# XuyangBai/D3Feat

Measured on NVIDIA H100. Metric: points/sec through KPFCNN encoder, higher is better.
Workload: dtype f32

## Files before the change

d3feat_b200/csrc/tc_common.cuh:

```cuda
#pragma once
#include "common.cuh"

namespace d3f {

__device__ __forceinline__ uint32_t smem_u32(const void* p) { return (uint32_t)__cvta_generic_to_shared(p); }

__device__ __forceinline__ void mbar_init(uint32_t bar, uint32_t count) {
  asm volatile("mbarrier.init.shared::cta.b64 [%0], %1;" ::"r"(bar), "r"(count) : "memory");
}
__device__ __forceinline__ void mbar_arrive(uint32_t bar) {
  asm volatile("mbarrier.arrive.shared::cta.b64 _, [%0];" ::"r"(bar) : "memory");
}
__device__ __forceinline__ void mbar_wait(uint32_t bar, uint32_t parity) {
  uint32_t ok;
  do {
    asm volatile(
        "{\n\t.reg .pred p;\n\t"
        "mbarrier.try_wait.parity.shared::cta.b64 p, [%1], %2;\n\t"
        "selp.u32 %0, 1, 0, p;\n\t}"
        : "=r"(ok)
        : "r"(bar), "r"(parity)
        : "memory");
  } while (!ok);
}
__device__ __forceinline__ void fence_proxy_async() { asm volatile("fence.proxy.async.shared::cta;" ::: "memory"); }

__device__ __forceinline__ uint64_t make_smem_desc(uint32_t saddr) {
  uint64_t d = 0;
  d |= (uint64_t)((saddr >> 4) & 0x3FFF);
  d |= (uint64_t)1 << 16;
  d |= (uint64_t)(1024 >> 4) << 32;
  d |= (uint64_t)1 << 62;
  return d;
}

__device__ __forceinline__ void wgmma_fence() { asm volatile("wgmma.fence.sync.aligned;" ::: "memory"); }
__device__ __forceinline__ void wgmma_commit() { asm volatile("wgmma.commit_group.sync.aligned;" ::: "memory"); }
template <int N>
__device__ __forceinline__ void wgmma_wait() { asm volatile("wgmma.wait_group.sync.aligned %0;" ::"n"(N) : "memory"); }
template <int R>
__device__ __forceinline__ void wgmma_reg_fence(float* d) {
#pragma unroll
  for (int i = 0; i < R; ++i) asm volatile("" : "+f"(d[i])::"memory");
}

template <int N>
__device__ __forceinline__ void wgmma_tf32(float* d, uint64_t adesc, uint64_t bdesc);
template <>
__device__ __forceinline__ void wgmma_tf32<32>(float* d, uint64_t adesc, uint64_t bdesc) {
  asm volatile(
      "{\n\t.reg .pred p;\n\tsetp.ne.b32 p, %18, 0;\n\t"
      "wgmma.mma_async.sync.aligned.m64n32k8.f32.tf32.tf32 "
      "{%0, %1, %2, %3, %4, %5, %6, %7, %8, %9, %10, %11, %12, %13, %14, %15}, %16, %17, p, 1, 1;\n\t}"
      : "+f"(d[0]), "+f"(d[1]), "+f"(d[2]), "+f"(d[3]), "+f"(d[4]), "+f"(d[5]), "+f"(d[6]), "+f"(d[7]), "+f"(d[8]), "+f"(d[9]), "+f"(d[10]), "+f"(d[11]), "+f"(d[12]), "+f"(d[13]), "+f"(d[14]), "+f"(d[15])
      : "l"(adesc), "l"(bdesc), "r"(1)
      : "memory");
}
template <>
__device__ __forceinline__ void wgmma_tf32<64>(float* d, uint64_t adesc, uint64_t bdesc) {
  asm volatile(
      "{\n\t.reg .pred p;\n\tsetp.ne.b32 p, %34, 0;\n\t"
      "wgmma.mma_async.sync.aligned.m64n64k8.f32.tf32.tf32 "
      "{%0, %1, %2, %3, %4, %5, %6, %7, %8, %9, %10, %11, %12, %13, %14, %15, %16, %17, %18, %19, %20, %21, %22, %23, %24, %25, %26, %27, %28, %29, %30, %31}, %32, %33, p, 1, 1;\n\t}"
      : "+f"(d[0]), "+f"(d[1]), "+f"(d[2]), "+f"(d[3]), "+f"(d[4]), "+f"(d[5]), "+f"(d[6]), "+f"(d[7]), "+f"(d[8]), "+f"(d[9]), "+f"(d[10]), "+f"(d[11]), "+f"(d[12]), "+f"(d[13]), "+f"(d[14]), "+f"(d[15]), "+f"(d[16]), "+f"(d[17]), "+f"(d[18]), "+f"(d[19]), "+f"(d[20]), "+f"(d[21]), "+f"(d[22]), "+f"(d[23]), "+f"(d[24]), "+f"(d[25]), "+f"(d[26]), "+f"(d[27]), "+f"(d[28]), "+f"(d[29]), "+f"(d[30]), "+f"(d[31])
      : "l"(adesc), "l"(bdesc), "r"(1)
      : "memory");
}
template <>
__device__ __forceinline__ void wgmma_tf32<96>(float* d, uint64_t adesc, uint64_t bdesc) {
  asm volatile(
      "{\n\t.reg .pred p;\n\tsetp.ne.b32 p, %50, 0;\n\t"
      "wgmma.mma_async.sync.aligned.m64n96k8.f32.tf32.tf32 "
      "{%0, %1, %2, %3, %4, %5, %6, %7, %8, %9, %10, %11, %12, %13, %14, %15, %16, %17, %18, %19, %20, %21, %22, %23, %24, %25, %26, %27, %28, %29, %30, %31, %32, %33, %34, %35, %36, %37, %38, %39, %40, %41, %42, %43, %44, %45, %46, %47}, %48, %49, p, 1, 1;\n\t}"
      : "+f"(d[0]), "+f"(d[1]), "+f"(d[2]), "+f"(d[3]), "+f"(d[4]), "+f"(d[5]), "+f"(d[6]), "+f"(d[7]), "+f"(d[8]), "+f"(d[9]), "+f"(d[10]), "+f"(d[11]), "+f"(d[12]), "+f"(d[13]), "+f"(d[14]), "+f"(d[15]), "+f"(d[16]), "+f"(d[17]), "+f"(d[18]), "+f"(d[19]), "+f"(d[20]), "+f"(d[21]), "+f"(d[22]), "+f"(d[23]), "+f"(d[24]), "+f"(d[25]), "+f"(d[26]), "+f"(d[27]), "+f"(d[28]), "+f"(d[29]), "+f"(d[30]), "+f"(d[31]), "+f"(d[32]), "+f"(d[33]), "+f"(d[34]), "+f"(d[35]), "+f"(d[36]), "+f"(d[37]), "+f"(d[38]), "+f"(d[39]), "+f"(d[40]), "+f"(d[41]), "+f"(d[42]), "+f"(d[43]), "+f"(d[44]), "+f"(d[45]), "+f"(d[46]), "+f"(d[47])
      : "l"(adesc), "l"(bdesc), "r"(1)
      : "memory");
}
template <>
__device__ __forceinline__ void wgmma_tf32<128>(float* d, uint64_t adesc, uint64_t bdesc) {
  asm volatile(
      "{\n\t.reg .pred p;\n\tsetp.ne.b32 p, %66, 0;\n\t"
      "wgmma.mma_async.sync.aligned.m64n128k8.f32.tf32.tf32 "
      "{%0, %1, %2, %3, %4, %5, %6, %7, %8, %9, %10, %11, %12, %13, %14, %15, %16, %17, %18, %19, %20, %21, %22, %23, %24, %25, %26, %27, %28, %29, %30, %31, %32, %33, %34, %35, %36, %37, %38, %39, %40, %41, %42, %43, %44, %45, %46, %47, %48, %49, %50, %51, %52, %53, %54, %55, %56, %57, %58, %59, %60, %61, %62, %63}, %64, %65, p, 1, 1;\n\t}"
      : "+f"(d[0]), "+f"(d[1]), "+f"(d[2]), "+f"(d[3]), "+f"(d[4]), "+f"(d[5]), "+f"(d[6]), "+f"(d[7]), "+f"(d[8]), "+f"(d[9]), "+f"(d[10]), "+f"(d[11]), "+f"(d[12]), "+f"(d[13]), "+f"(d[14]), "+f"(d[15]), "+f"(d[16]), "+f"(d[17]), "+f"(d[18]), "+f"(d[19]), "+f"(d[20]), "+f"(d[21]), "+f"(d[22]), "+f"(d[23]), "+f"(d[24]), "+f"(d[25]), "+f"(d[26]), "+f"(d[27]), "+f"(d[28]), "+f"(d[29]), "+f"(d[30]), "+f"(d[31]), "+f"(d[32]), "+f"(d[33]), "+f"(d[34]), "+f"(d[35]), "+f"(d[36]), "+f"(d[37]), "+f"(d[38]), "+f"(d[39]), "+f"(d[40]), "+f"(d[41]), "+f"(d[42]), "+f"(d[43]), "+f"(d[44]), "+f"(d[45]), "+f"(d[46]), "+f"(d[47]), "+f"(d[48]), "+f"(d[49]), "+f"(d[50]), "+f"(d[51]), "+f"(d[52]), "+f"(d[53]), "+f"(d[54]), "+f"(d[55]), "+f"(d[56]), "+f"(d[57]), "+f"(d[58]), "+f"(d[59]), "+f"(d[60]), "+f"(d[61]), "+f"(d[62]), "+f"(d[63])
      : "l"(adesc), "l"(bdesc), "r"(1)
      : "memory");
}

__device__ __forceinline__ float4 lds128(uint32_t addr) {
  float4 v;
  asm volatile("ld.shared.v4.f32 {%0, %1, %2, %3}, [%4];" : "=f"(v.x), "=f"(v.y), "=f"(v.z), "=f"(v.w) : "r"(addr));
  return v;
}
__device__ __forceinline__ void sts128(uint32_t addr, float4 v) {
  asm volatile("st.shared.v4.f32 [%0], {%1, %2, %3, %4};" ::"r"(addr), "f"(v.x), "f"(v.y), "f"(v.z), "f"(v.w) : "memory");
}
__device__ __forceinline__ float lds32(uint32_t addr) {
  float v;
  asm volatile("ld.shared.f32 %0, [%1];" : "=f"(v) : "r"(addr));
  return v;
}
__device__ __forceinline__ void sts32(uint32_t addr, float v) {
  asm volatile("st.shared.f32 [%0], %1;" ::"r"(addr), "f"(v) : "memory");
}

__device__ __forceinline__ void split_tf32(float x, float& hi, float& lo) {
  hi = __uint_as_float((__float_as_uint(x) + 0x1000u) & 0xFFFFE000u);
  lo = x - hi;
}

__device__ __forceinline__ void tma_bulk_g2s(uint32_t dst_smem, const void* src, uint32_t bytes, uint32_t bar) {
  asm volatile("cp.async.bulk.shared::cluster.global.mbarrier::complete_tx::bytes [%0], [%1], %2, [%3];"
               ::"r"(dst_smem), "l"(src), "r"(bytes), "r"(bar) : "memory");
}
__device__ __forceinline__ void mbar_arrive_expect_tx(uint32_t bar, uint32_t bytes) {
  asm volatile("mbarrier.arrive.expect_tx.shared::cta.b64 _, [%0], %1;" ::"r"(bar), "r"(bytes) : "memory");
}
__device__ __forceinline__ void cp_async16(uint32_t dst_smem, const void* src) {
  asm volatile("cp.async.cg.shared.global [%0], [%1], 16;" ::"r"(dst_smem), "l"(src) : "memory");
}
__device__ __forceinline__ void cp_async16_zfill(uint32_t dst_smem, const void* src, bool valid) {
  const int sz = valid ? 16 : 0;
  asm volatile("cp.async.cg.shared.global [%0], [%1], 16, %2;" ::"r"(dst_smem), "l"(src), "r"(sz) : "memory");
}

}
```

d3feat_b200/csrc/tc_gemm.cu:

```cuda
#include <stdlib.h>

#include "ops.cuh"
#include "tc_common.cuh"

namespace d3f {

constexpr int kTcBM = 128;
constexpr int kTcBK = 32;
constexpr int kTcProducerThreads = 128;
constexpr int kTcConsumerWarps = 8;
constexpr int kTcThreads = kTcProducerThreads + 32 * kTcConsumerWarps;

__global__ void __launch_bounds__(256) pack_weight_kernel(const float* __restrict__ W, int K, int N, int Kpad,
                                                          int Npad, float* __restrict__ packed) {
  long long total = (long long)Npad * Kpad;
  for (long long i = (long long)blockIdx.x * blockDim.x + threadIdx.x; i < total; i += (long long)gridDim.x * blockDim.x) {
    int k = (int)(i / Npad), n = (int)(i % Npad);
    float x = (n < N && k < K) ? W[(size_t)k * N + n] : 0.f;
    float hi, lo;
    split_tf32(x, hi, lo);
    int kc = k >> 5, kl = k & 31;
    size_t slab = (size_t)kc * 2 * Npad * 32;
    size_t off = (size_t)n * 32 + (size_t)((((kl >> 2) ^ (n & 7)) << 2) | (kl & 3));
    packed[slab + off] = hi;
    packed[slab + (size_t)Npad * 32 + off] = lo;
  }
}

int tc_padded_k(int K) { return (K + kTcBK - 1) / kTcBK * kTcBK; }
int tc_block_n(int N) { return N > 64 ? 128 : (N > 32 ? 64 : 32); }
int tc_padded_n(int N) { int bn = tc_block_n(N); return (N + bn - 1) / bn * bn; }
size_t tc_packed_floats(int K, int N) { return 2 * (size_t)tc_padded_k(K) * tc_padded_n(N); }

int tc_pack_weight(const float* W, int K, int N, float* packed, cudaStream_t stream) {
  D3F_REQUIRE(K >= 1 && N >= 1 && W && packed, D3F_ERR_INVALID, "pack_weight: bad arguments");
  int Kpad = tc_padded_k(K), Npad = tc_padded_n(N);
  long long total = (long long)Npad * Kpad;
  int blocks = (int)min((total + 255) / 256, (long long)kNumSMs * 8);
  pack_weight_kernel<<<blocks, 256, 0, stream>>>(W, K, N, Kpad, Npad, packed);
  D3F_LAUNCH_CHECK("pack_weight_kernel");
  return D3F_OK;
}

template <int BN>
struct TcSmem {
  static constexpr int kStages = BN >= 128 ? 3 : 4;
  static constexpr int kABytes = kTcBM * 128;
  static constexpr int kBBytes = BN * 128;
  static constexpr int kStageBytes = 2 * kABytes + 2 * kBBytes;
  static constexpr int kTotal = kStages * kStageBytes + 1024  + 256 ;
  static_assert(kTotal <= 232448, "shared memory budget of an H100 SM (227 KB)");
};

template <int BN>
__global__ void __launch_bounds__(kTcThreads, 1)
tc_gemm_kernel(const float* __restrict__ A, const float* __restrict__ A2, int K1, const float* __restrict__ Bp,
               float* __restrict__ C, int Mcap, int N, int K, int Kpad, int Npad, int chunks_per_split, Epilogue ep) {
  const int M = ep.m_dev ? min(Mcap, max(__ldg(ep.m_dev) - ep.m_off, 0)) : Mcap;
  const int ntn = Npad / BN;
  const int tiles = ceil_div(M, kTcBM) * ntn;
  if ((int)blockIdx.x >= tiles) return;
  const int my_tiles = (tiles - (int)blockIdx.x + (int)gridDim.x - 1) / (int)gridDim.x;
  extern __shared__ uint8_t smem_raw[];
  using S = TcSmem<BN>;
  constexpr int kStages = S::kStages;
  uint8_t* smem = (uint8_t*)(((uintptr_t)smem_raw + 1023) & ~(uintptr_t)1023);
  uint64_t* full = (uint64_t*)(smem + kStages * S::kStageBytes);
  uint64_t* empty = full + kStages;

  const int tid = threadIdx.x, warp = tid >> 5, lane = tid & 31;
  const int kt0 = blockIdx.z * chunks_per_split;
  const int nk = min(Kpad / kTcBK - kt0, chunks_per_split);
  C += (size_t)blockIdx.z * Mcap * N;

  if (tid == 0) {
    for (int s = 0; s < kStages; ++s) {
      mbar_init(smem_u32(&full[s]), kTcProducerThreads + 1);
      mbar_init(smem_u32(&empty[s]), kTcConsumerWarps);
    }
    asm volatile("fence.mbarrier_init.release.cluster;" ::: "memory");
  }
  __syncthreads();

  if (warp < 4) {
    const int chunk = tid & 7;
    const int rsub = tid >> 3;
    const int total = my_tiles * nk;
    int i_tile = (int)blockIdx.x, i_kt = 0, i_g = 0;
    auto issue_chunk = [&]() {
      const int s = i_g % kStages;
      mbar_wait(smem_u32(&empty[s]), ((uint32_t)(i_g / kStages) & 1u) ^ 1u);
      uint8_t* st = smem + s * S::kStageBytes;
      const int m0 = (i_tile / ntn) * kTcBM, n0 = (i_tile % ntn) * BN;
      int k0 = (kt0 + i_kt) * kTcBK + chunk * 4;
      const float* src = A;
      int ld = K;
      if (A2 != nullptr) {
        ld = K1;
        if (k0 >= K1) {
          src = A2;
          ld = K - K1;
          k0 -= K1;
        }
      }
#pragma unroll
      for (int it = 0; it < kTcBM / 16; ++it) {
        const int row = it * 16 + rsub;
        const int gm = m0 + row;
        const uint32_t off = (uint32_t)row * 128u + (uint32_t)((chunk ^ (row & 7)) << 4);
        const bool ok = gm < M && k0 < ld;
        cp_async16_zfill(smem_u32(st + off), src + (size_t)(ok ? gm : 0) * ld + (ok ? k0 : 0), ok);
      }
      if (tid == 0) {
        const uint32_t fb = smem_u32(&full[s]);
        const float* slab = Bp + (size_t)(kt0 + i_kt) * 2 * Npad * 32 + (size_t)n0 * 32;
        mbar_arrive_expect_tx(fb, 2u * S::kBBytes);
        tma_bulk_g2s(smem_u32(st + 2 * S::kABytes), slab, S::kBBytes, fb);
        tma_bulk_g2s(smem_u32(st + 2 * S::kABytes + S::kBBytes), slab + (size_t)Npad * 32, S::kBBytes, fb);
      }
      ++i_g;
      if (++i_kt == nk) {
        i_kt = 0;
        i_tile += (int)gridDim.x;
      }
    };
    for (int i = 0; i < kStages - 1; ++i) {
      if (i < total) issue_chunk();
      asm volatile("cp.async.commit_group;" ::: "memory");
    }
    for (int g = 0; g < total; ++g) {
      const int s = g % kStages;
      asm volatile("cp.async.wait_group %0;" ::"n"(kStages - 2) : "memory");
      const uint32_t st_s = smem_u32(smem + s * S::kStageBytes);
      float4 x[kTcBM / 16];
#pragma unroll
      for (int it = 0; it < kTcBM / 16; ++it) {
        const int row = it * 16 + rsub;
        x[it] = lds128(st_s + (uint32_t)row * 128u + (uint32_t)((chunk ^ (row & 7)) << 4));
      }
#pragma unroll
      for (int it = 0; it < kTcBM / 16; ++it) {
        const int row = it * 16 + rsub;
        const uint32_t off = (uint32_t)row * 128u + (uint32_t)((chunk ^ (row & 7)) << 4);
        float4 hi, lo;
        split_tf32(x[it].x, hi.x, lo.x);
        split_tf32(x[it].y, hi.y, lo.y);
        split_tf32(x[it].z, hi.z, lo.z);
        split_tf32(x[it].w, hi.w, lo.w);
        sts128(st_s + off, hi);
        sts128(st_s + S::kABytes + off, lo);
      }
      fence_proxy_async();
      mbar_arrive(smem_u32(&full[s]));
      if (i_g < total) issue_chunk();
      asm volatile("cp.async.commit_group;" ::: "memory");
    }
  } else {
    constexpr int R = BN / 2;
    const int cw = (warp - 4) >> 2;
    const int wq = warp & 3;
    const bool has_bn = ep.bn_scale != nullptr, has_bias = ep.bias != nullptr, has_res = ep.residual != nullptr;
    const bool has_leaky = ep.leaky_alpha >= 0.f;
    const bool pairs = (N & 1) == 0;
    float acc[R], sum[R];
    int g = 0;
    for (int i = 0; i < my_tiles; ++i) {
      const int t = (int)blockIdx.x + i * (int)gridDim.x;
      const int m0 = (t / ntn) * kTcBM, n0 = (t % ntn) * BN;
#pragma unroll
      for (int j = 0; j < R; ++j) sum[j] = 0.f;
      for (int kt = 0; kt < nk; ++kt, ++g) {
        const int s = g % kStages;
        mbar_wait(smem_u32(&full[s]), (uint32_t)(g / kStages) & 1u);
#pragma unroll
        for (int j = 0; j < R; ++j) acc[j] = 0.f;
        wgmma_fence();
        const uint32_t sa = smem_u32(smem + s * S::kStageBytes);
        const uint64_t a_hi = make_smem_desc(sa + (uint32_t)cw * (64 * 128));
        const uint64_t a_lo = make_smem_desc(sa + S::kABytes + (uint32_t)cw * (64 * 128));
        const uint64_t b_hi = make_smem_desc(sa + 2 * S::kABytes), b_lo = make_smem_desc(sa + 2 * S::kABytes + S::kBBytes);
#pragma unroll
        for (int j = 0; j < kTcBK / 8; ++j) {
          const uint64_t adv = (uint64_t)((j * 32) >> 4);
          wgmma_tf32<BN>(acc, a_hi + adv, b_hi + adv);
          wgmma_tf32<BN>(acc, a_lo + adv, b_hi + adv);
          wgmma_tf32<BN>(acc, a_hi + adv, b_lo + adv);
        }
        wgmma_commit();
        wgmma_wait<0>();
        wgmma_reg_fence<R>(acc);
        __syncwarp();
        if (lane == 0) mbar_arrive(smem_u32(&empty[s]));
#pragma unroll
        for (int j = 0; j < R; ++j) sum[j] += acc[j];
      }

#pragma unroll
      for (int h = 0; h < 2; ++h) {
        const int gm = m0 + 64 * cw + 16 * wq + (lane >> 2) + 8 * h;
        if (gm >= M) continue;
        const float rs = ep.rowscale != nullptr ? ep.rowscale[gm] : 1.f;
        const size_t orow = ep.row_map ? (size_t)ep.row_map[gm] : (size_t)gm;
        float* crow = C + orow * N;
        const float* rrow = has_res ? ep.residual + orow * N : nullptr;
#pragma unroll
        for (int j = 0; j < BN / 8; ++j) {
          const int gn = n0 + 8 * j + 2 * (lane & 3);
          if (gn >= N) continue;
          const bool both = gn + 1 < N;
          float y[2] = {sum[4 * j + 2 * h] * rs, sum[4 * j + 2 * h + 1] * rs};
          float r[2] = {0.f, 0.f};
          if (has_res) {
            if (pairs && both) {
              const float2 rv = *reinterpret_cast<const float2*>(rrow + gn);
              r[0] = rv.x;
              r[1] = rv.y;
            } else {
              r[0] = rrow[gn];
              if (both) r[1] = rrow[gn + 1];
            }
          }
#pragma unroll
          for (int e = 0; e < 2; ++e) {
            const int n = both ? gn + e : gn;
            if (has_bn) y[e] = fmaf(y[e], ep.bn_scale[n], ep.bn_shift[n]);
            if (has_bias) y[e] += ep.bias[n];
            y[e] += r[e];
            if (has_leaky) y[e] = y[e] > 0.f ? y[e] : y[e] * ep.leaky_alpha;
          }
          if (pairs && both) {
            *reinterpret_cast<float2*>(crow + gn) = make_float2(y[0], y[1]);
          } else {
            crow[gn] = y[0];
            if (both) crow[gn + 1] = y[1];
          }
        }
      }
    }
  }
}

__global__ void __launch_bounds__(256) splitk_reduce_kernel(const float* __restrict__ part, int splits, int Mcap, int N,
                                                            Epilogue ep, float* __restrict__ C) {
  const int M = ep.m_dev ? min(Mcap, max(__ldg(ep.m_dev) - ep.m_off, 0)) : Mcap;
  const long long slab = (long long)Mcap * N;
  long long total = (long long)M * N;
  for (long long i = (long long)blockIdx.x * blockDim.x + threadIdx.x; i < total; i += (long long)gridDim.x * blockDim.x) {
    int m = (int)(i / N), n = (int)(i % N);
    float y = 0.f;
    for (int z = 0; z < splits; ++z) y += part[(size_t)z * slab + i];
    if (ep.rowscale) y *= ep.rowscale[m];
    if (ep.bn_scale) y = fmaf(y, ep.bn_scale[n], ep.bn_shift[n]);
    if (ep.bias) y += ep.bias[n];
    const size_t orow = ep.row_map ? (size_t)ep.row_map[m] : (size_t)m;
    if (ep.residual) y += ep.residual[orow * N + n];
    if (ep.leaky_alpha >= 0.f) y = y > 0.f ? y : y * ep.leaky_alpha;
    C[orow * N + n] = y;
  }
}

template <int BN>
static int launch_tc(const float* A, const float* A2, int K1, const float* Bp, float* C, int M, int N, int K,
                     const Epilogue& ep, cudaStream_t stream, int splits, float* split_ws, bool persistent) {
  using S = TcSmem<BN>;
  static bool configured = false;
  if (!configured) {
    D3F_CUDA(cudaFuncSetAttribute(tc_gemm_kernel<BN>, cudaFuncAttributeMaxDynamicSharedMemorySize, S::kTotal));
    configured = true;
  }
  const int Kpad = tc_padded_k(K), Npad = tc_padded_n(N);
  const int nk = Kpad / kTcBK;
  const int tiles = ceil_div(M, kTcBM) * (Npad / BN);
  if (splits <= 1) {
    const int grid = persistent && tiles > kNumSMs ? kNumSMs : tiles;
    tc_gemm_kernel<BN><<<grid, kTcThreads, S::kTotal, stream>>>(A, A2, K1, Bp, C, M, N, K, Kpad, Npad, nk, ep);
    D3F_LAUNCH_CHECK("tc_gemm_kernel");
    return D3F_OK;
  }
  const int cps = ceil_div(nk, splits);
  splits = ceil_div(nk, cps);
  Epilogue raw;
  raw.rowscale = nullptr; raw.bn_scale = nullptr; raw.bn_shift = nullptr; raw.bias = nullptr; raw.residual = nullptr;
  raw.leaky_alpha = -1.f; raw.row_map = nullptr; raw.m_dev = ep.m_dev; raw.m_off = ep.m_off;
  dim3 grid(tiles, 1, splits);
  tc_gemm_kernel<BN><<<grid, kTcThreads, S::kTotal, stream>>>(A, A2, K1, Bp, split_ws, M, N, K, Kpad, Npad, cps, raw);
  D3F_LAUNCH_CHECK("tc_gemm_kernel");
  long long total = (long long)M * N;
  int blocks = (int)min((total + 255) / 256, (long long)kNumSMs * 8);
  splitk_reduce_kernel<<<blocks, 256, 0, stream>>>(split_ws, splits, M, N, ep, C);
  D3F_LAUNCH_CHECK("splitk_reduce_kernel");
  return D3F_OK;
}

static int env_int(const char* name, int dflt) {
  const char* v = getenv(name);
  return v ? atoi(v) : dflt;
}

bool tc_gemm_supported(const float* A, int K) {
  return (K % 4 == 0) && ((reinterpret_cast<uintptr_t>(A) & 15) == 0);
}

int tc_gemm_splits(int M, int N, int K) {
  const int bn = tc_block_n(N);
  const long long ctas = (long long)ceil_div(M, kTcBM) * (tc_padded_n(N) / bn);
  const int nk = tc_padded_k(K) / kTcBK;
  if (ctas >= 96 || nk < 16) return 1;
  int best = 1;
  long long best_cost = (long long)ceil_div((int)ctas, kNumSMs) * nk * 8;
  for (int s = 2; s <= 8 && s <= nk / 4; ++s) {
    const int cps = ceil_div(nk, s);
    const int eff = ceil_div(nk, cps);
    if (eff != s) continue;
    long long cost = (long long)ceil_div((int)(ctas * s), kNumSMs) * cps * 8 + 40 + 6 * s;
    if (cost < best_cost) {
      best_cost = cost;
      best = s;
    }
  }
  return best;
}
size_t tc_gemm_split_ws_floats(int M, int N, int K) {
  const int bn = tc_block_n(N);
  const long long ctas = (long long)ceil_div(M, kTcBM) * (tc_padded_n(N) / bn);
  const int nk = tc_padded_k(K) / kTcBK;
  if (nk < 16) return 0;
  const long long tiles = ctas < 95 ? ctas : 95;
  return (size_t)(8 * tiles * kTcBM * bn);
}

int tc_gemm(const float* A, const float* Bp, float* C, int M, int N, int K, const Epilogue& ep, cudaStream_t stream,
            float* split_ws, const float* A2, int K1) {
  if (M <= 0 || N <= 0) return D3F_OK;
  D3F_REQUIRE(tc_gemm_supported(A, K), D3F_ERR_INVALID, "tc_gemm: needs K %% 4 == 0 and 16-byte aligned A");
  if (A2 != nullptr)
    D3F_REQUIRE(K1 > 0 && K1 < K && K1 % kTcBK == 0 && tc_gemm_supported(A2, K - K1), D3F_ERR_INVALID,
                "tc_gemm: split A operand needs K1 %% %d == 0 and a 16-byte aligned second matrix", kTcBK);
  int bn = tc_block_n(N);
  if (bn == 128 && K <= 256 && M >= 8192) bn = 64;
  const int splits = split_ws != nullptr ? tc_gemm_splits(M, N, K) : 1;
  const bool persistent = splits <= 1 && (tc_padded_k(K) / kTcBK <= 4 || env_int("D3F_TC_STREAM", 0) != 0);
  switch (bn) {
    case 128: return launch_tc<128>(A, A2, K1, Bp, C, M, N, K, ep, stream, splits, split_ws, persistent);
    case 64: return launch_tc<64>(A, A2, K1, Bp, C, M, N, K, ep, stream, splits, split_ws, persistent);
    default: return launch_tc<32>(A, A2, K1, Bp, C, M, N, K, ep, stream, splits, split_ws, persistent);
  }
}

}
```

Baseline: 56.91 million.

## Load A via TMA and split TF32 in registers using register-sourced WGMMA

Replaces the 128-thread cp.async producer, which also split A into hi/lo TF32 halves in shared memory, with a single-thread TMA producer that loads A through a 2D tensor map with 128B swizzle. Consumers now read A fragments from shared memory, split them into hi/lo in registers, and issue register-sourced WGMMA (3xTF32), pipelining fragment loads against the async MMAs. This halves the A footprint per stage, drops the producer's smem read/write pass, and lets smaller-BN configs run two CTAs per SM. In exchange it adds tensor-map encoding on the host per launch, per-thread split work on the consumers, and relies on tensor-map OOB zero-fill for M/K edges.

```diff
diff --git a/d3feat_b200/csrc/tc_common.cuh b/d3feat_b200/csrc/tc_common.cuh
--- a/d3feat_b200/csrc/tc_common.cuh
+++ b/d3feat_b200/csrc/tc_common.cuh
@@ -87,6 +87,39 @@
       : "memory");
 }
 
+template <int N>
+__device__ __forceinline__ void wgmma_tf32_rs(float* d, const uint32_t* a, uint64_t bdesc);
+template <>
+__device__ __forceinline__ void wgmma_tf32_rs<32>(float* d, const uint32_t* a, uint64_t bdesc) {
+  asm volatile(
+      "{\n\t.reg .pred p;\n\tsetp.ne.b32 p, %21, 0;\n\t"
+      "wgmma.mma_async.sync.aligned.m64n32k8.f32.tf32.tf32 "
+      "{%0, %1, %2, %3, %4, %5, %6, %7, %8, %9, %10, %11, %12, %13, %14, %15}, {%16, %17, %18, %19}, %20, p, 1, 1;\n\t}"
+      : "+f"(d[0]), "+f"(d[1]), "+f"(d[2]), "+f"(d[3]), "+f"(d[4]), "+f"(d[5]), "+f"(d[6]), "+f"(d[7]), "+f"(d[8]), "+f"(d[9]), "+f"(d[10]), "+f"(d[11]), "+f"(d[12]), "+f"(d[13]), "+f"(d[14]), "+f"(d[15])
+      : "r"(a[0]), "r"(a[1]), "r"(a[2]), "r"(a[3]), "l"(bdesc), "r"(1)
+      : "memory");
+}
+template <>
+__device__ __forceinline__ void wgmma_tf32_rs<64>(float* d, const uint32_t* a, uint64_t bdesc) {
+  asm volatile(
+      "{\n\t.reg .pred p;\n\tsetp.ne.b32 p, %37, 0;\n\t"
+      "wgmma.mma_async.sync.aligned.m64n64k8.f32.tf32.tf32 "
+      "{%0, %1, %2, %3, %4, %5, %6, %7, %8, %9, %10, %11, %12, %13, %14, %15, %16, %17, %18, %19, %20, %21, %22, %23, %24, %25, %26, %27, %28, %29, %30, %31}, {%32, %33, %34, %35}, %36, p, 1, 1;\n\t}"
+      : "+f"(d[0]), "+f"(d[1]), "+f"(d[2]), "+f"(d[3]), "+f"(d[4]), "+f"(d[5]), "+f"(d[6]), "+f"(d[7]), "+f"(d[8]), "+f"(d[9]), "+f"(d[10]), "+f"(d[11]), "+f"(d[12]), "+f"(d[13]), "+f"(d[14]), "+f"(d[15]), "+f"(d[16]), "+f"(d[17]), "+f"(d[18]), "+f"(d[19]), "+f"(d[20]), "+f"(d[21]), "+f"(d[22]), "+f"(d[23]), "+f"(d[24]), "+f"(d[25]), "+f"(d[26]), "+f"(d[27]), "+f"(d[28]), "+f"(d[29]), "+f"(d[30]), "+f"(d[31])
+      : "r"(a[0]), "r"(a[1]), "r"(a[2]), "r"(a[3]), "l"(bdesc), "r"(1)
+      : "memory");
+}
+template <>
+__device__ __forceinline__ void wgmma_tf32_rs<128>(float* d, const uint32_t* a, uint64_t bdesc) {
+  asm volatile(
+      "{\n\t.reg .pred p;\n\tsetp.ne.b32 p, %69, 0;\n\t"
+      "wgmma.mma_async.sync.aligned.m64n128k8.f32.tf32.tf32 "
+      "{%0, %1, %2, %3, %4, %5, %6, %7, %8, %9, %10, %11, %12, %13, %14, %15, %16, %17, %18, %19, %20, %21, %22, %23, %24, %25, %26, %27, %28, %29, %30, %31, %32, %33, %34, %35, %36, %37, %38, %39, %40, %41, %42, %43, %44, %45, %46, %47, %48, %49, %50, %51, %52, %53, %54, %55, %56, %57, %58, %59, %60, %61, %62, %63}, {%64, %65, %66, %67}, %68, p, 1, 1;\n\t}"
+      : "+f"(d[0]), "+f"(d[1]), "+f"(d[2]), "+f"(d[3]), "+f"(d[4]), "+f"(d[5]), "+f"(d[6]), "+f"(d[7]), "+f"(d[8]), "+f"(d[9]), "+f"(d[10]), "+f"(d[11]), "+f"(d[12]), "+f"(d[13]), "+f"(d[14]), "+f"(d[15]), "+f"(d[16]), "+f"(d[17]), "+f"(d[18]), "+f"(d[19]), "+f"(d[20]), "+f"(d[21]), "+f"(d[22]), "+f"(d[23]), "+f"(d[24]), "+f"(d[25]), "+f"(d[26]), "+f"(d[27]), "+f"(d[28]), "+f"(d[29]), "+f"(d[30]), "+f"(d[31]), "+f"(d[32]), "+f"(d[33]), "+f"(d[34]), "+f"(d[35]), "+f"(d[36]), "+f"(d[37]), "+f"(d[38]), "+f"(d[39]), "+f"(d[40]), "+f"(d[41]), "+f"(d[42]), "+f"(d[43]), "+f"(d[44]), "+f"(d[45]), "+f"(d[46]), "+f"(d[47]), "+f"(d[48]), "+f"(d[49]), "+f"(d[50]), "+f"(d[51]), "+f"(d[52]), "+f"(d[53]), "+f"(d[54]), "+f"(d[55]), "+f"(d[56]), "+f"(d[57]), "+f"(d[58]), "+f"(d[59]), "+f"(d[60]), "+f"(d[61]), "+f"(d[62]), "+f"(d[63])
+      : "r"(a[0]), "r"(a[1]), "r"(a[2]), "r"(a[3]), "l"(bdesc), "r"(1)
+      : "memory");
+}
+
 __device__ __forceinline__ float4 lds128(uint32_t addr) {
   float4 v;
   asm volatile("ld.shared.v4.f32 {%0, %1, %2, %3}, [%4];" : "=f"(v.x), "=f"(v.y), "=f"(v.z), "=f"(v.w) : "r"(addr));
@@ -113,6 +146,10 @@
   asm volatile("cp.async.bulk.shared::cluster.global.mbarrier::complete_tx::bytes [%0], [%1], %2, [%3];"
                ::"r"(dst_smem), "l"(src), "r"(bytes), "r"(bar) : "memory");
 }
+__device__ __forceinline__ void tma_load_2d(uint32_t dst_smem, const void* tmap, int x, int y, uint32_t bar) {
+  asm volatile("cp.async.bulk.tensor.2d.shared::cluster.global.mbarrier::complete_tx::bytes [%0], [%1, {%2, %3}], [%4];"
+               ::"r"(dst_smem), "l"(tmap), "r"(x), "r"(y), "r"(bar) : "memory");
+}
 __device__ __forceinline__ void mbar_arrive_expect_tx(uint32_t bar, uint32_t bytes) {
   asm volatile("mbarrier.arrive.expect_tx.shared::cta.b64 _, [%0], %1;" ::"r"(bar), "r"(bytes) : "memory");
 }
diff --git a/d3feat_b200/csrc/tc_gemm.cu b/d3feat_b200/csrc/tc_gemm.cu
--- a/d3feat_b200/csrc/tc_gemm.cu
+++ b/d3feat_b200/csrc/tc_gemm.cu
@@ -1,3 +1,5 @@
+#include <cuda.h>
+#include <cudaTypedefs.h>
 #include <stdlib.h>
 
 #include "ops.cuh"
@@ -7,9 +9,8 @@
 
 constexpr int kTcBM = 128;
 constexpr int kTcBK = 32;
-constexpr int kTcProducerThreads = 128;
 constexpr int kTcConsumerWarps = 8;
-constexpr int kTcThreads = kTcProducerThreads + 32 * kTcConsumerWarps;
+constexpr int kTcThreads = 32 * kTcConsumerWarps + 32;
 
 __global__ void __launch_bounds__(256) pack_weight_kernel(const float* __restrict__ W, int K, int N, int Kpad,
                                                           int Npad, float* __restrict__ packed) {
@@ -44,23 +45,24 @@
 
 template <int BN>
 struct TcSmem {
-  static constexpr int kStages = BN >= 128 ? 3 : 4;
+  static constexpr int kCtasPerSm = BN >= 128 ? 1 : 2;
+  static constexpr int kStages = BN >= 64 ? 3 : 4;
   static constexpr int kABytes = kTcBM * 128;
   static constexpr int kBBytes = BN * 128;
-  static constexpr int kStageBytes = 2 * kABytes + 2 * kBBytes;
+  static constexpr int kStageBytes = kABytes + 2 * kBBytes;
   static constexpr int kTotal = kStages * kStageBytes + 1024  + 256 ;
-  static_assert(kTotal <= 232448, "shared memory budget of an H100 SM (227 KB)");
+  static_assert(kCtasPerSm * (kTotal + 1024) <= 233472, "shared memory of an H100 SM (228 KB, 1 KB reserved per CTA)");
 };
 
 template <int BN>
-__global__ void __launch_bounds__(kTcThreads, 1)
-tc_gemm_kernel(const float* __restrict__ A, const float* __restrict__ A2, int K1, const float* __restrict__ Bp,
-               float* __restrict__ C, int Mcap, int N, int K, int Kpad, int Npad, int chunks_per_split, Epilogue ep) {
+__global__ void __launch_bounds__(kTcThreads, TcSmem<BN>::kCtasPerSm)
+tc_gemm_kernel(const __grid_constant__ CUtensorMap tmA, const __grid_constant__ CUtensorMap tmA2, int K1,
+               const float* __restrict__ Bp, float* __restrict__ C, int Mcap, int N, int Kpad, int Npad,
+               int chunks_per_split, Epilogue ep) {
   const int M = ep.m_dev ? min(Mcap, max(__ldg(ep.m_dev) - ep.m_off, 0)) : Mcap;
   const int ntn = Npad / BN;
   const int tiles = ceil_div(M, kTcBM) * ntn;
   if ((int)blockIdx.x >= tiles) return;
-  const int my_tiles = (tiles - (int)blockIdx.x + (int)gridDim.x - 1) / (int)gridDim.x;
   extern __shared__ uint8_t smem_raw[];
   using S = TcSmem<BN>;
   constexpr int kStages = S::kStages;
@@ -75,118 +77,88 @@
 
   if (tid == 0) {
     for (int s = 0; s < kStages; ++s) {
-      mbar_init(smem_u32(&full[s]), kTcProducerThreads + 1);
+      mbar_init(smem_u32(&full[s]), 1);
       mbar_init(smem_u32(&empty[s]), kTcConsumerWarps);
     }
     asm volatile("fence.mbarrier_init.release.cluster;" ::: "memory");
   }
   __syncthreads();
 
-  if (warp < 4) {
-    const int chunk = tid & 7;
-    const int rsub = tid >> 3;
-    const int total = my_tiles * nk;
-    int i_tile = (int)blockIdx.x, i_kt = 0, i_g = 0;
-    auto issue_chunk = [&]() {
-      const int s = i_g % kStages;
-      mbar_wait(smem_u32(&empty[s]), ((uint32_t)(i_g / kStages) & 1u) ^ 1u);
-      uint8_t* st = smem + s * S::kStageBytes;
-      const int m0 = (i_tile / ntn) * kTcBM, n0 = (i_tile % ntn) * BN;
-      int k0 = (kt0 + i_kt) * kTcBK + chunk * 4;
-      const float* src = A;
-      int ld = K;
-      if (A2 != nullptr) {
-        ld = K1;
-        if (k0 >= K1) {
-          src = A2;
-          ld = K - K1;
-          k0 -= K1;
+  if (warp == kTcConsumerWarps) {
+    if (lane == 0) {
+      const int total = (tiles - (int)blockIdx.x + (int)gridDim.x - 1) / (int)gridDim.x * nk;
+      int tile = (int)blockIdx.x, kt = 0;
+      for (int g = 0; g < total; ++g) {
+        const int s = g % kStages;
+        mbar_wait(smem_u32(&empty[s]), ((uint32_t)(g / kStages) & 1u) ^ 1u);
+        const uint32_t st = smem_u32(smem + s * S::kStageBytes);
+        const uint32_t fb = smem_u32(&full[s]);
+        const int m0 = (tile / ntn) * kTcBM, n0 = (tile % ntn) * BN;
+        const int k0 = (kt0 + kt) * kTcBK;
+        mbar_arrive_expect_tx(fb, (uint32_t)S::kStageBytes);
+        if (k0 < K1)
+          tma_load_2d(st, &tmA, k0, m0, fb);
+        else
+          tma_load_2d(st, &tmA2, k0 - K1, m0, fb);
+        const float* slab = Bp + (size_t)(kt0 + kt) * 2 * Npad * 32 + (size_t)n0 * 32;
+        tma_bulk_g2s(st + S::kABytes, slab, S::kBBytes, fb);
+        tma_bulk_g2s(st + S::kABytes + S::kBBytes, slab + (size_t)Npad * 32, S::kBBytes, fb);
+        if (++kt == nk) {
+          kt = 0;
+          tile += (int)gridDim.x;
         }
       }
-#pragma unroll
-      for (int it = 0; it < kTcBM / 16; ++it) {
-        const int row = it * 16 + rsub;
-        const int gm = m0 + row;
-        const uint32_t off = (uint32_t)row * 128u + (uint32_t)((chunk ^ (row & 7)) << 4);
-        const bool ok = gm < M && k0 < ld;
-        cp_async16_zfill(smem_u32(st + off), src + (size_t)(ok ? gm : 0) * ld + (ok ? k0 : 0), ok);
-      }
-      if (tid == 0) {
-        const uint32_t fb = smem_u32(&full[s]);
-        const float* slab = Bp + (size_t)(kt0 + i_kt) * 2 * Npad * 32 + (size_t)n0 * 32;
-        mbar_arrive_expect_tx(fb, 2u * S::kBBytes);
-        tma_bulk_g2s(smem_u32(st + 2 * S::kABytes), slab, S::kBBytes, fb);
-        tma_bulk_g2s(smem_u32(st + 2 * S::kABytes + S::kBBytes), slab + (size_t)Npad * 32, S::kBBytes, fb);
-      }
-      ++i_g;
-      if (++i_kt == nk) {
-        i_kt = 0;
-        i_tile += (int)gridDim.x;
-      }
-    };
-    for (int i = 0; i < kStages - 1; ++i) {
-      if (i < total) issue_chunk();
-      asm volatile("cp.async.commit_group;" ::: "memory");
-    }
-    for (int g = 0; g < total; ++g) {
-      const int s = g % kStages;
-      asm volatile("cp.async.wait_group %0;" ::"n"(kStages - 2) : "memory");
-      const uint32_t st_s = smem_u32(smem + s * S::kStageBytes);
-      float4 x[kTcBM / 16];
-#pragma unroll
-      for (int it = 0; it < kTcBM / 16; ++it) {
-        const int row = it * 16 + rsub;
-        x[it] = lds128(st_s + (uint32_t)row * 128u + (uint32_t)((chunk ^ (row & 7)) << 4));
-      }
-#pragma unroll
-      for (int it = 0; it < kTcBM / 16; ++it) {
-        const int row = it * 16 + rsub;
-        const uint32_t off = (uint32_t)row * 128u + (uint32_t)((chunk ^ (row & 7)) << 4);
-        float4 hi, lo;
-        split_tf32(x[it].x, hi.x, lo.x);
-        split_tf32(x[it].y, hi.y, lo.y);
-        split_tf32(x[it].z, hi.z, lo.z);
-        split_tf32(x[it].w, hi.w, lo.w);
-        sts128(st_s + off, hi);
-        sts128(st_s + S::kABytes + off, lo);
-      }
-      fence_proxy_async();
-      mbar_arrive(smem_u32(&full[s]));
-      if (i_g < total) issue_chunk();
-      asm volatile("cp.async.commit_group;" ::: "memory");
     }
   } else {
     constexpr int R = BN / 2;
-    const int cw = (warp - 4) >> 2;
+    const int cw = warp >> 2;
     const int wq = warp & 3;
+    const int r0 = 64 * cw + 16 * wq + (lane >> 2);
+    const uint32_t a_row = (uint32_t)r0 * 128u + (uint32_t)(lane & 3) * 4u, a_swz = (uint32_t)(r0 & 7);
+    auto load_a = [&](float* x, uint32_t sa, int j) {
+#pragma unroll
+      for (int q = 0; q < 4; ++q)
+        x[q] = lds32(sa + a_row + (uint32_t)(q & 1) * 1024u + ((((uint32_t)(2 * j + (q >> 1))) ^ a_swz) << 4));
+    };
     const bool has_bn = ep.bn_scale != nullptr, has_bias = ep.bias != nullptr, has_res = ep.residual != nullptr;
     const bool has_leaky = ep.leaky_alpha >= 0.f;
     const bool pairs = (N & 1) == 0;
     float acc[R], sum[R];
     int g = 0;
-    for (int i = 0; i < my_tiles; ++i) {
-      const int t = (int)blockIdx.x + i * (int)gridDim.x;
+    for (int t = (int)blockIdx.x; t < tiles; t += (int)gridDim.x) {
       const int m0 = (t / ntn) * kTcBM, n0 = (t % ntn) * BN;
 #pragma unroll
       for (int j = 0; j < R; ++j) sum[j] = 0.f;
       for (int kt = 0; kt < nk; ++kt, ++g) {
         const int s = g % kStages;
         mbar_wait(smem_u32(&full[s]), (uint32_t)(g / kStages) & 1u);
+        const uint32_t sa = smem_u32(smem + s * S::kStageBytes);
+        const uint64_t b_hi = make_smem_desc(sa + S::kABytes), b_lo = make_smem_desc(sa + S::kABytes + S::kBBytes);
+        float x[4];
+        uint32_t ah[2][4], al[2][4];
+        load_a(x, sa, 0);
 #pragma unroll
         for (int j = 0; j < R; ++j) acc[j] = 0.f;
-        wgmma_fence();
-        const uint32_t sa = smem_u32(smem + s * S::kStageBytes);
-        const uint64_t a_hi = make_smem_desc(sa + (uint32_t)cw * (64 * 128));
-        const uint64_t a_lo = make_smem_desc(sa + S::kABytes + (uint32_t)cw * (64 * 128));
-        const uint64_t b_hi = make_smem_desc(sa + 2 * S::kABytes), b_lo = make_smem_desc(sa + 2 * S::kABytes + S::kBBytes);
 #pragma unroll
         for (int j = 0; j < kTcBK / 8; ++j) {
+          uint32_t* h = ah[j & 1];
+          uint32_t* l = al[j & 1];
+#pragma unroll
+          for (int q = 0; q < 4; ++q) {
+            float hi, lo;
+            split_tf32(x[q], hi, lo);
+            h[q] = __float_as_uint(hi);
+            l[q] = __float_as_uint(lo);
+          }
           const uint64_t adv = (uint64_t)((j * 32) >> 4);
-          wgmma_tf32<BN>(acc, a_hi + adv, b_hi + adv);
-          wgmma_tf32<BN>(acc, a_lo + adv, b_hi + adv);
-          wgmma_tf32<BN>(acc, a_hi + adv, b_lo + adv);
+          wgmma_fence();
+          wgmma_tf32_rs<BN>(acc, h, b_hi + adv);
+          wgmma_tf32_rs<BN>(acc, l, b_hi + adv);
+          wgmma_tf32_rs<BN>(acc, h, b_lo + adv);
+          wgmma_commit();
+          if (j + 1 < kTcBK / 8) load_a(x, sa, j + 1);
+          wgmma_wait<1>();
         }
-        wgmma_commit();
         wgmma_wait<0>();
         wgmma_reg_fence<R>(acc);
         __syncwarp();
@@ -194,7 +166,6 @@
 #pragma unroll
         for (int j = 0; j < R; ++j) sum[j] += acc[j];
       }
-
 #pragma unroll
       for (int h = 0; h < 2; ++h) {
         const int gm = m0 + 64 * cw + 16 * wq + (lane >> 2) + 8 * h;
@@ -259,6 +230,27 @@
   }
 }
 
+static int encode_a_map(CUtensorMap* map, const float* A, int rows, int cols) {
+  static PFN_cuTensorMapEncodeTiled_v12000 encode = nullptr;
+  if (encode == nullptr) {
+    void* fn = nullptr;
+    cudaDriverEntryPointQueryResult q;
+    D3F_CUDA(cudaGetDriverEntryPoint("cuTensorMapEncodeTiled", &fn, cudaEnableDefault, &q));
+    D3F_REQUIRE(q == cudaDriverEntryPointSuccess && fn != nullptr, D3F_ERR_CUDA,
+                "tc_gemm: the driver has no cuTensorMapEncodeTiled");
+    encode = reinterpret_cast<PFN_cuTensorMapEncodeTiled_v12000>(fn);
+  }
+  const cuuint64_t dims[2] = {(cuuint64_t)cols, (cuuint64_t)rows};
+  const cuuint64_t strides[1] = {(cuuint64_t)cols * sizeof(float)};
+  const cuuint32_t box[2] = {(cuuint32_t)kTcBK, (cuuint32_t)kTcBM};
+  const cuuint32_t elem[2] = {1, 1};
+  const CUresult r = encode(map, CU_TENSOR_MAP_DATA_TYPE_FLOAT32, 2, const_cast<float*>(A), dims, strides, box, elem,
+                            CU_TENSOR_MAP_INTERLEAVE_NONE, CU_TENSOR_MAP_SWIZZLE_128B, CU_TENSOR_MAP_L2_PROMOTION_L2_256B,
+                            CU_TENSOR_MAP_FLOAT_OOB_FILL_NONE);
+  D3F_REQUIRE(r == CUDA_SUCCESS, D3F_ERR_CUDA, "tc_gemm: cuTensorMapEncodeTiled failed (%d)", (int)r);
+  return D3F_OK;
+}
+
 template <int BN>
 static int launch_tc(const float* A, const float* A2, int K1, const float* Bp, float* C, int M, int N, int K,
                      const Epilogue& ep, cudaStream_t stream, int splits, float* split_ws, bool persistent) {
@@ -271,9 +263,21 @@
   const int Kpad = tc_padded_k(K), Npad = tc_padded_n(N);
   const int nk = Kpad / kTcBK;
   const int tiles = ceil_div(M, kTcBM) * (Npad / BN);
+  CUtensorMap tmA, tmA2;
+  if (A2 != nullptr) {
+    int rc = encode_a_map(&tmA, A, M, K1);
+    if (rc == D3F_OK) rc = encode_a_map(&tmA2, A2, M, K - K1);
+    if (rc != D3F_OK) return rc;
+  } else {
+    const int rc = encode_a_map(&tmA, A, M, K);
+    if (rc != D3F_OK) return rc;
+    tmA2 = tmA;
+    K1 = Kpad;
+  }
   if (splits <= 1) {
-    const int grid = persistent && tiles > kNumSMs ? kNumSMs : tiles;
-    tc_gemm_kernel<BN><<<grid, kTcThreads, S::kTotal, stream>>>(A, A2, K1, Bp, C, M, N, K, Kpad, Npad, nk, ep);
+    const int cap = kNumSMs * S::kCtasPerSm;
+    const int grid = persistent && tiles > cap ? cap : tiles;
+    tc_gemm_kernel<BN><<<grid, kTcThreads, S::kTotal, stream>>>(tmA, tmA2, K1, Bp, C, M, N, Kpad, Npad, nk, ep);
     D3F_LAUNCH_CHECK("tc_gemm_kernel");
     return D3F_OK;
   }
@@ -283,7 +287,7 @@
   raw.rowscale = nullptr; raw.bn_scale = nullptr; raw.bn_shift = nullptr; raw.bias = nullptr; raw.residual = nullptr;
   raw.leaky_alpha = -1.f; raw.row_map = nullptr; raw.m_dev = ep.m_dev; raw.m_off = ep.m_off;
   dim3 grid(tiles, 1, splits);
-  tc_gemm_kernel<BN><<<grid, kTcThreads, S::kTotal, stream>>>(A, A2, K1, Bp, split_ws, M, N, K, Kpad, Npad, cps, raw);
+  tc_gemm_kernel<BN><<<grid, kTcThreads, S::kTotal, stream>>>(tmA, tmA2, K1, Bp, split_ws, M, N, Kpad, Npad, cps, raw);
   D3F_LAUNCH_CHECK("tc_gemm_kernel");
   long long total = (long long)M * N;
   int blocks = (int)min((total + 255) / 256, (long long)kNumSMs * 8);
```

New measurement: 61.58 million, median of 6. 1.08x the previous value.
